# jakovdev/SequenceAligner

Hardware: AMD Instinct MI355X
Metric: pair-alignments/sec (higher is better)
Workload: dtype u16x2; 1 GPU; cfg2: 10000 protein seqs x U[80,120], nw blosum62 {'gap_pen': 4}, all-vs-all packed triangular; pairs=49995000, cells=501594494441, parallelism=pair-range x1

## Files before the change

sequencealigner_amd/csrc/sa_context.hip:

```cpp
#include <algorithm>
#include <cmath>
#include <cstdio>
#include <cstdlib>
#include <cstring>

#include "sa_ctx.h"

bool sa_device_ready(int device)
{
	int count = 0;
	hipError_t err = hipGetDeviceCount(&count);
	if (err != hipSuccess || count <= 0) {
		sa_set_error("No HIP devices available (%s); libseqalign_hip has no CPU fallback",
			     err == hipSuccess ? "device count is 0" : hipGetErrorString(err));
		return false;
	}
	if (device < 0 || device >= count) {
		sa_set_error("HIP device %d out of range (%d visible)", device, count);
		return false;
	}
	SA_HIP_CHECK(hipSetDevice(device), return false);
	return true;
}

// ... 234 lines not shown
}

extern "C" sa_ctx *sa_ctx_create(int device, struct sa_input in, const struct sa_scoring *sc)
{
	return sa_guard("sa_ctx_create", (sa_ctx *)nullptr, [&] { return ctx_create_impl(device, in, sc); });
}

extern "C" void sa_ctx_destroy(sa_ctx *ctx)
{
	if (!ctx)
		return;
	(void)hipSetDevice(ctx->device);
	for (auto &ev : ctx->events) {
		(void)hipEventDestroy(ev.e0);
		(void)hipEventDestroy(ev.e1);
	}
	sa_plan_release(ctx);
	sa_deliver_release(ctx);
	for (auto &ar : ctx->arranged) {
		(void)hipFree(ar.d_codes);
		(void)hipFree(ar.d_off);
		(void)hipFree(ar.d_rowmap);
		(void)hipFree(ar.d_posmap);
	}
	(void)hipFree(ctx->d_codes);
	(void)hipFree(ctx->d_meta);
	(void)hipFree(ctx->d_off);
	(void)hipFree(ctx->d_sub);
	(void)hipFree(ctx->d_sub8);
	(void)hipFree(ctx->d_scratch);
	(void)hipFree(ctx->d_counters);
	for (hipEvent_t ev : ctx->slot_done)
		if (ev)
			(void)hipEventDestroy(ev);
	(void)hipFree(ctx->d_long_scratch);
	for (int k = 0; k < sa_ctx::NSIDE; k++) {
		if (ctx->side[k])
			(void)hipStreamDestroy(ctx->side[k]);
		if (ctx->join_ev[k])
			(void)hipEventDestroy(ctx->join_ev[k]);
	}
	if (ctx->fork_ev)
		(void)hipEventDestroy(ctx->fork_ev);
	delete ctx;
}

// ... 32 lines not shown
	do {
		SA_HIP_CHECK(hipMalloc(&ar.d_codes, codes_s.size()), break);
		SA_HIP_CHECK(hipMalloc(&ar.d_off, sizeof(int32_t) * off_s.size()), break);
		SA_HIP_CHECK(hipMalloc(&ar.d_rowmap, sizeof(int32_t) * rowmap.size()), break);
		SA_HIP_CHECK(hipMalloc(&ar.d_posmap, sizeof(int32_t) * posmap.size()), break);
		SA_HIP_CHECK(hipMemcpy(ar.d_codes, codes_s.data(), codes_s.size(), hipMemcpyHostToDevice), break);
		SA_HIP_CHECK(hipMemcpy(ar.d_off, off_s.data(), sizeof(int32_t) * off_s.size(), hipMemcpyHostToDevice), break);
		SA_HIP_CHECK(hipMemcpy(ar.d_rowmap, rowmap.data(), sizeof(int32_t) * rowmap.size(), hipMemcpyHostToDevice), break);
		SA_HIP_CHECK(hipMemcpy(ar.d_posmap, posmap.data(), sizeof(int32_t) * posmap.size(), hipMemcpyHostToDevice), break);
		ctx->arranged.push_back(ar);
		ok = true;
	} while (0);
	if (!ok) {
		(void)hipFree(ar.d_codes);
		(void)hipFree(ar.d_off);
		(void)hipFree(ar.d_rowmap);
		(void)hipFree(ar.d_posmap);
		return false;
	}
	*out = &ctx->arranged.back();
	return true;
}

extern "C" void sa_ctx_timing(sa_ctx *ctx, int enable)
{
	if (!ctx)
		return;
	(void)hipSetDevice(ctx->device);
	for (auto &ev : ctx->events) {
		(void)hipEventDestroy(ev.e0);
		(void)hipEventDestroy(ev.e1);
	}
	ctx->events.clear();
	ctx->timing = enable != 0;
}

static int timing_read_impl(sa_ctx *ctx, char *kernel_name, int cap, int64_t *launches, double *total_ms,
			    int64_t *pairs, int64_t *cells, double *all_kernels_ms)
{
	if (!ctx)
		return 1;
	(void)hipSetDevice(ctx->device);
	struct Acc {
		double ms = 0;
		int64_t n = 0, pairs = 0, cells = 0;
	};
// ... 45 lines not shown
```

sequencealigner_amd/csrc/sa_ctx.h:

```cpp
#ifndef SA_CTX_H
#define SA_CTX_H

#include <atomic>
#include <chrono>
#include <deque>
#include <exception>
#include <memory>
#include <new>
#include <string>
#include <vector>

#include "sa_env.h"
#include "sa_guard.h"
#include "sa_internal.h"
#include "sa_plan.h"

struct sa_ctx {
	int device = 0;
	int32_t num = 0, max_len = 0, min_len = 0;
	int64_t pairs = 0;
	sa_scoring sc{};
	SaEnv env;
	std::vector<sa_meta> meta;
	std::vector<int32_t> off;
// ... 10 lines not shown
	unsigned *d_counters = nullptr;
	uint64_t call_no = 0;
	hipEvent_t slot_done[COUNTER_SLOTS] = {};
	bool slot_dirty[COUNTER_SLOTS] = {};
	int32_t *d_long_scratch = nullptr;
	int64_t long_stride = 0;
	int long_wgs = 0;
	int persistent_wgs = 0;
	enum { NSIDE = 8 };
	hipStream_t side[NSIDE] = {};
	hipEvent_t fork_ev = nullptr, join_ev[NSIDE] = {};
	bool sys_ok = false;
	int32_t sys_pconst = 0, sys_q = 0;
	int64_t sys_gain = 0, sys_slack = 0;
	int pk_kmax = 0, pk16_kmax = 0;
	int pk16_f16_kmax = 0;
	int pk_chunk_cap = SA_SYS_CHUNK;
	int32_t pk_pconst = 0, pk_q = 0, pk_floor = 0;
	int64_t pk_gain = 0, pk_slack = 0, pk_extra = 0;
	struct Arranged {
		SaArrKey key;
		uint8_t *d_codes = nullptr;
		int32_t *d_off = nullptr, *d_rowmap = nullptr, *d_posmap = nullptr;
	};
	std::deque<Arranged> arranged;
	bool out_is_host = false;
	struct Plan {
		SaHostPlan h;
		struct DevClass {
			int32_t *d_jlist = nullptr, *d_tprefix = nullptr, *d_tlist = nullptr;
			int64_t *d_doff = nullptr;
		};
		struct DevBundle {
			SaPkClassArgs *d_args = nullptr;
			uint32_t *d_ulist = nullptr;
		};
		std::vector<DevClass> dc;
		std::vector<DevBundle> db;
		SaPlaceSeg *d_segs = nullptr;
		int32_t nsegs = 0;
		uint64_t stamp = 0;
	};
	std::vector<std::unique_ptr<Plan>> plans;
	Plan *plan = nullptr;
	uint64_t plan_clock = 0;
	bool timing = false;
// ... 13 lines not shown
		double encode = 0, device = 0, upload = 0, code_objects = 0, pin = 0, plan = 0, arrange = 0;
	} setup;
	struct Deliver {
		hipStream_t compute = nullptr, copy = nullptr;
		hipEvent_t done[2] = {}, copied[2] = {};
		int32_t *d_buf[2] = {};
		int64_t buf_elems[2] = {};
		int32_t *h_stage[2] = {};
		int64_t stage_elems[2] = {};
		int32_t *d_packed = nullptr, *d_full = nullptr;
		int64_t packed_elems = 0, full_elems = 0;
		unsigned *h_counters = nullptr;
		int64_t h_counters_n = 0;
	} dl;
};

static inline double sa_ms_since(std::chrono::steady_clock::time_point t0)
{
	return std::chrono::duration<double, std::milli>(std::chrono::steady_clock::now() - t0).count();
}

bool sa_device_ready(int device);
bool sa_arranged_store(sa_ctx *ctx, const SaArrKey &key, const sa_ctx::Arranged **out);
SaPlanInputs sa_plan_inputs(const sa_ctx *ctx);

void sa_plan_release(sa_ctx *ctx);
bool sa_plan_get(sa_ctx *ctx, int64_t start, int64_t count, int world, bool share_host);
bool sa_prepare_range(sa_ctx *ctx, int64_t start, int64_t count, bool host_out);
int sa_align_range_impl(sa_ctx *ctx, int64_t start, int64_t count, int32_t *d_scores, void *stream, bool out16,
			int world = 0, int rank = 0, int32_t *host_out = nullptr);

void sa_deliver_release(sa_ctx *ctx);
bool sa_host_range_is_pinned(const void *p, size_t bytes);
size_t sa_host_available_bytes();
bool sa_host_range_in_malloc_heap(const void *p, size_t bytes);

bool sa_progress_wanted();
void sa_report_progress(double fraction);
void sa_progress_speaker(bool here);
int sa_devices_in_use(const SaEnv &env);

bool sa_align_gathered(struct sa_input in, struct sa_output out, const struct sa_scoring *sc, const int *devices, int ndev,
		       double *phase_seconds, double *breakdown_ms);
bool sa_rccl_available(std::string *why);

#endif
// ... 1 lines not shown
```

sequencealigner_amd/csrc/sa_env.cpp:

```cpp
#include "sa_env.h"

#include <algorithm>
#include <cstdlib>

static bool flag(const char *name) { return getenv(name) != nullptr; }
static int number(const char *name, int fallback, int lo, int hi)
{
	const char *v = getenv(name);
	if (!v || !*v)
		return fallback;
	return std::max(lo, std::min(hi, atoi(v)));
}

SaEnv sa_env_read()
{
	SaEnv e;
	e.force_generic = flag("SA_HIP_FORCE_GENERIC");
	e.no_pk = flag("SA_HIP_NO_PK");
	e.no_pk16 = flag("SA_HIP_NO_PK16");
	e.no_sort = flag("SA_HIP_NO_SORT");
	e.concurrent_classes = flag("SA_HIP_CONCURRENT_CLASSES");
	e.one_tile_size = flag("SA_HIP_ONE_TILE_SIZE");
	e.chunk = number("SA_HIP_CHUNK", 0, 1, 32);
	e.pk_wgs = number("SA_HIP_PK_WGS", 0, 0, 1 << 20);
	e.stagger = number("SA_HIP_STAGGER", 0, 0, 64);
	e.rotate_prio = getenv("SA_HIP_ROTATE_PRIO") ? (atoi(getenv("SA_HIP_ROTATE_PRIO")) != 0) : -1;
	e.small_below = number("SA_HIP_SMALL_BELOW", 16, 0, 1 << 20);
	e.small_div = number("SA_HIP_SMALL_DIV", 4, 2, 64);
	e.small_frac = number("SA_HIP_SMALL_FRAC", 5, 2, 1 << 20);
	e.no_pin = flag("SA_HIP_NO_PIN");
	e.no_direct = flag("SA_HIP_NO_DIRECT");
	e.no_shells = flag("SA_HIP_NO_SHELLS");
	e.devices = number("SA_HIP_DEVICES", 0, 0, 1024);
	e.split = number("SA_HIP_SPLIT", 0, 0, 1024);
	e.gather = getenv("SA_HIP_GATHER") ? (atoi(getenv("SA_HIP_GATHER")) != 0) : -1;
	e.tiles_split = number("SA_HIP_TILES_SPLIT", 0, 0, 64);
	e.verbose = flag("SA_HIP_VERBOSE");
	e.stamps = flag("SA_HIP_STAMPS");
	e.stamps_dump = getenv("SA_HIP_STAMPS_DUMP");
	e.ztrace = flag("SA_HIP_ZTRACE");
	return e;
}
```

sequencealigner_amd/csrc/sa_env.h:

```cpp
#ifndef SA_ENV_H
#define SA_ENV_H

struct SaEnv {
	bool force_generic = false;
	bool no_pk = false;
	bool no_pk16 = false;
	bool no_sort = false;
	bool concurrent_classes = false;
	bool one_tile_size = false;
	int chunk = 0;
	int pk_wgs = 0;
	int stagger = 0;
	int rotate_prio = -1;
	int small_below = 16;
	int small_div = 4;
	int small_frac = 5;
	bool no_pin = false;
	bool no_direct = false;
	bool no_shells = false;
	int devices = 0;
	int split = 0;
	int gather = -1;
	int tiles_split = 0;
	bool verbose = false;
	bool stamps = false;
	const char *stamps_dump = nullptr;
	bool ztrace = false;
};

SaEnv sa_env_read();
// ... 3 lines not shown
```

sequencealigner_amd/csrc/sa_launch.hip:

```cpp
#include <algorithm>
#include <cstdio>
#include <cstring>

#include "sa_ctx.h"


static void plan_free_device(sa_ctx::Plan &pl)
{
	for (auto &c : pl.dc) {
		(void)hipFree(c.d_jlist);
		(void)hipFree(c.d_tprefix);
		(void)hipFree(c.d_tlist);
		(void)hipFree(c.d_doff);
	}
	(void)hipFree(pl.d_segs);
	for (auto &b : pl.db) {
		(void)hipFree(b.d_args);
		(void)hipFree(b.d_ulist);
	}
	pl.dc.clear();
	pl.db.clear();
	pl.d_segs = nullptr;
}

void sa_plan_release(sa_ctx *ctx)
{
	for (auto &pl : ctx->plans)
		plan_free_device(*pl);
	ctx->plans.clear();
	ctx->plan = nullptr;
}

template <typename T> static bool upload(T *&dst, const std::vector<T> &v)
{
	SA_HIP_CHECK(hipMalloc(reinterpret_cast<void **>(&dst), sizeof(T) * std::max<size_t>(v.size(), 1)), return false);
	if (!v.empty()) {
		SA_HIP_CHECK(hipMemcpy(dst, v.data(), sizeof(T) * v.size(), hipMemcpyHostToDevice), return false);
	}
	return true;
}

static bool resolve_levels(sa_ctx *ctx, const SaArrKey (&keys)[SA_PK_SORT_LEVELS], SaArranged (&lv)[SA_PK_SORT_LEVELS])
{
	for (int l = 0; l < SA_PK_SORT_LEVELS; l++) {
		lv[l] = SaArranged{};
		if (!keys[l].block)
			continue;
		const sa_ctx::Arranged *ar = nullptr;
		if (!sa_arranged_store(ctx, keys[l], &ar))
			return false;
		if (ar)
			lv[l] = { ar->d_codes, ar->d_off, ar->d_rowmap, ar->d_posmap, ar->key.block };
	}
	return true;
}

static bool plan_upload(sa_ctx *ctx, sa_ctx::Plan &pl)
{
	const SaHostPlan &h = pl.h;
	pl.dc.resize(h.classes.size());
	for (size_t ci = 0; ci < h.classes.size(); ci++) {
		const auto &cl = h.classes[ci];
		auto &d = pl.dc[ci];
		if (!upload(d.d_jlist, cl.jlist) || !upload(d.d_tprefix, cl.tprefix))
			return false;
		if (h.world >= 1 && (!upload(d.d_tlist, cl.tlist) || !upload(d.d_doff, cl.doff)))
			return false;
	}
	if (h.world >= 1 && !h.segs.empty()) {
		std::vector<SaPlaceSeg> segs(h.segs.size());
		for (size_t k = 0; k < h.segs.size(); k++) {
			const SaHostSeg &hs = h.segs[k];
			SaPlaceSeg &sg = segs[k];
			sg = SaPlaceSeg{};
			sg.src = hs.src;
// ... 7 lines not shown
			if (hs.map_kind) {
				const sa_ctx::Arranged *ar = nullptr;
				if (!sa_arranged_store(ctx, hs.key, &ar))
					return false;
				if (!ar) {
					sa_set_error("plan: placement names an arranged copy the store does not have");
					return false;
				}
				sg.map = hs.map_kind == 2 ? ar->d_posmap : ar->d_rowmap;
			}
		}
		if (!upload(pl.d_segs, segs))
			return false;
		pl.nsegs = (int32_t)segs.size();
	}
	pl.db.resize(h.bundles.size());
	for (size_t bi = 0; bi < h.bundles.size(); bi++) {
		const auto &b = h.bundles[bi];
		std::vector<SaPkClassArgs> args(b.args.size());
		for (size_t x = 0; x < b.args.size(); x++) {
			const SaHostPkArgs &ha = b.args[x];
			SaPkClassArgs &a = args[x];
			a = SaPkClassArgs{};
			if (!resolve_levels(ctx, ha.lv, a.lv))
				return false;
			const auto &d = pl.dc[(size_t)ha.cls_index];
			a.jlist = d.d_jlist;
			a.tprefix = d.d_tprefix;
			a.dense_off = h.world >= 1 ? d.d_doff : nullptr;
			a.ncols = ha.ncols;
			a.npart = ha.npart;
			a.k = ha.k;
			a.delta = ha.delta;
			a.pk_base = ha.pk_base;
			a.chunk = ha.chunk;
		}
		if (!upload(pl.db[bi].d_args, args) || !upload(pl.db[bi].d_ulist, b.ulist))
			return false;
	}
	return true;
}

bool sa_plan_get(sa_ctx *ctx, int64_t start, int64_t count, int world, bool share_host)
{
	for (auto &pl : ctx->plans)
		if (pl->h.start == start && pl->h.count == count && pl->h.world == world && pl->h.share_host == share_host) {
			pl->stamp = ++ctx->plan_clock;
// ... 511 lines not shown
```

sequencealigner_amd/csrc/sa_plan.cpp:

```cpp
#include "sa_plan.h"
#include "sa_guard.h"

#include <algorithm>
#include <cmath>
#include <cstdlib>

int32_t sa_column_of(int64_t p)
{
	int64_t j = (int64_t)((1.0 + std::sqrt(1.0 + 8.0 * (double)p)) * 0.5);
	while (j * (j - 1) / 2 > p)
		--j;
	while ((j + 1) * j / 2 <= p)
		++j;
	return (int32_t)j;
}

SaPairPlan::SaPairPlan(const sa_meta *m, int32_t n) : num(n), pairs((int64_t)n * (n - 1) / 2), meta(m)
{
	len_prefix.assign((size_t)n + 1, 0);
	cell_prefix.assign((size_t)n + 1, 0);
	for (int32_t k = 0; k < n; k++) {
		len_prefix[(size_t)k + 1] = len_prefix[(size_t)k] + m[k].len;
		cell_prefix[(size_t)k + 1] = cell_prefix[(size_t)k] + (int64_t)m[k].len * len_prefix[(size_t)k];
	}
// ... 82 lines not shown
	for (int32_t b0 = 0; b0 + block <= num; b0 += block) {
		for (int32_t k = 0; k < block; k++)
			idx[(size_t)k] = b0 + k;
		std::stable_sort(idx.begin(), idx.end(), [&](int32_t a, int32_t b) { return meta[a].len > meta[b].len; });
		rounds.clear();
		rest.clear();
		for (int32_t k = 0; k < block;) {
			int32_t e = k;
			while (e < block && meta[idx[(size_t)e]].len == meta[idx[(size_t)k]].len)
				e++;
			const int32_t pure = (e - k) / ng * ng;
			rounds.insert(rounds.end(), idx.begin() + k, idx.begin() + k + pure);
			rest.insert(rest.end(), idx.begin() + k + pure, idx.begin() + e);
			k = e;
		}
		rounds.insert(rounds.end(), rest.begin(), rest.end());
		for (int32_t r = 0; r < block / ng; r++) {
			const int32_t pass = r / slots, w = r % slots;
			const int32_t slot = (pass & 1) ? slots - 1 - w : w;
			for (int g = 0; g < ng; g++) {
				const int gg = (pass & 1) ? ng - 1 - g : g;
				rowmap[(size_t)(b0 + slot * wave_rows + gg * ch + pass)] = rounds[(size_t)(r * ng + g)];
			}
		}
	}
}

static const char *const TOO_LARGE = "packed range too large for one launch; split it into smaller ranges";

bool sa_plan_host(const SaPlanInputs &in, int64_t start, int64_t count, int world, bool share_host, SaHostPlan &plan)
{
	plan = SaHostPlan();
	const int32_t num = in.num;
	const int64_t all_pairs = (int64_t)num * (num - 1) / 2;
	if (num < 2 || !in.meta || start < 0 || count <= 0 || start > all_pairs - count || world < 0 || world > 1024) {
		sa_set_error("plan: bad range [%lld,+%lld) of %lld pairs or world %d", (long long)start, (long long)count,
			     (long long)all_pairs, world);
		return false;
	}
	const int64_t end = start + count;
	std::vector<std::vector<int32_t>> jl((size_t)SA_PLAN_NCLASSES), tp((size_t)SA_PLAN_NCLASSES);
	std::vector<int64_t> cpairs((size_t)SA_PLAN_NCLASSES, 0), ccells((size_t)SA_PLAN_NCLASSES, 0);
	std::vector<std::vector<std::pair<int32_t, int32_t>>> rows_of((size_t)SA_PLAN_NCLASSES);
	std::vector<int64_t> lenpre((size_t)num + 1, 0);
	for (int32_t k = 0; k < num; k++)
		lenpre[(size_t)k + 1] = lenpre[(size_t)k] + in.meta[k].len;
// ... 414 lines not shown
```

sequencealigner_amd/csrc/sa_plan.h:

```cpp
#ifndef SA_PLAN_H
#define SA_PLAN_H

#include <cstdint>
#include <string>
#include <utility>
#include <vector>

#include "sa_shapes.h"

int32_t sa_column_of(int64_t p);
inline int64_t sa_tri(int64_t j) { return j * (j - 1) / 2; }

struct SaPairPlan {
	int32_t num = 0;
	int64_t pairs = 0;
	const sa_meta *meta = nullptr;
	std::vector<int64_t> len_prefix;
	std::vector<int64_t> cell_prefix;
	SaPairPlan(const sa_meta *m, int32_t n);
	int64_t cells_before(int64_t p) const;
};

struct SaArrKey {
	int ng = 0, ch = 0;
// ... 23 lines not shown
	bool sys_ok = false;
	int32_t sys_pconst = 0, sys_q = 0;
	int64_t sys_gain = 0, sys_slack = 0;
	int pk_kmax = 0, pk16_kmax = 0, pk16_f16_kmax = 0, pk_chunk_cap = SA_SYS_CHUNK;
	int32_t pk_pconst = 0, pk_q = 0, pk_floor = 0;
	int64_t pk_gain = 0, pk_slack = 0, pk_extra = 0;
};
SaKernelLimits sa_kernel_limits(const sa_scoring &sc, int32_t max_len, int32_t min_len, bool force_generic, bool no_pk, bool no_pk16);

int32_t sa_pk_delta(const SaPlanInputs &in, int g, int k);
int32_t sa_pk_base(const SaPlanInputs &in, int g, int k);

struct SaPkCls {
	bool small;
	int g, k;
};
SaPkCls sa_pk_decode(int cls);
int sa_systolic_class_for(int32_t n);

bool sa_arranged_exists(int32_t num, const SaArrKey &key);
int sa_pk_arranged_keys(const SaPlanInputs &in, int pk_g, int pk_k, int32_t chunk_pk, bool host_out, SaArrKey (&lv)[SA_PK_SORT_LEVELS]);
void sa_arrange_rows(const sa_meta *meta, int32_t num, const SaArrKey &key, std::vector<int32_t> &rowmap);

struct SaHostClass {
	int cls = 0;
	int32_t ncols = 0, ntiles = 0;
	int32_t npart = 0;
	int32_t chunk = 0;
	int64_t pairs = 0, cells = 0;
	std::vector<int32_t> jlist, tprefix;
	std::vector<int32_t> part_rows;
	std::vector<int32_t> tlist;
	std::vector<int64_t> doff;
	std::vector<int16_t> owner;
	std::vector<int32_t> rank_first;
	std::vector<int64_t> rank_pairs, rank_cells;
};

struct SaHostSeg {
	int64_t src, dst;
	int32_t count, pos0, ia, ib, flags;
	int map_kind;
	SaArrKey key;
};

struct SaHostPkArgs {
// ... 39 lines not shown
```

sequencealigner_amd/csrc/sa_shapes.h:

```cpp
#ifndef SA_SHAPES_H
#define SA_SHAPES_H

#include <cstdint>

#include "../../include/seqalign_hip.h"

#if defined(__HIPCC__)
#define SA_HD __host__ __device__
#else
#define SA_HD
#endif

enum : int { SA_CODE_SEP = 24, SA_CODE_NOP = 25, SA_CODE_ROWS = 26 };

void sa_set_error(const char *fmt, ...) __attribute__((format(printf, 1, 2)));


#define SA_SYS_CHUNK 32
#define SA_SYS_WPB(G, LONG) ((G) >= 32 ? 4 : 1)
#define SA_SYS_CLASS_LIST(X) \
	X(0, 8, 1) X(1, 8, 2) X(2, 8, 3) X(3, 8, 4) \
	X(4, 8, 5) X(5, 8, 6) X(6, 8, 7) X(7, 8, 8) \
	X(8, 8, 9) X(9, 8, 10) X(10, 8, 11) X(11, 8, 12) \
	X(12, 8, 13) X(13, 8, 14) X(14, 8, 15) X(15, 8, 16) \
// ... 29 lines not shown
#define SA_PK_K_LIST(X) \
	X(1) X(2) X(3) X(4) X(5) X(6) X(7) X(8) X(9) X(10) X(11) X(12) \
	X(13) X(14) X(15) X(16) X(17) X(18) X(19) X(20) X(21) X(22) X(23) X(24)
#define SA_PK_K16_MIN 13
#define SA_PK16_KMAX 64
#define SA_PK16_F16_KMAX 52
#define SA_PK_K16_LIST(X) \
	X(13) X(14) X(15) X(16) X(17) X(18) X(19) X(20) X(21) X(22) X(23) X(24) X(25) X(26) \
	X(27) X(28) X(29) X(30) X(31) X(32) X(33) X(34) X(35) X(36) X(37) X(38) X(39) X(40) \
	X(41) X(42) X(43) X(44) X(45) X(46) X(47) X(48) X(49) X(50) X(51) X(52) X(53) X(54) \
	X(55) X(56) X(57) X(58) X(59) X(60) X(61) X(62) X(63) X(64)
enum : int { SA_PK_CLASS0 = SA_SYS_NCLASSES + 1, SA_PK16_CLASS0 = SA_PK_CLASS0 + SA_PK_KMAX + 1,
	     SA_PK_CLASSES_END = SA_PK16_CLASS0 + SA_PK16_KMAX + 1,
	     SA_PK_SMALL = SA_PK_CLASSES_END - SA_PK_CLASS0,
	     SA_PLAN_NCLASSES = SA_PK_CLASSES_END + SA_PK_SMALL };

#define SA_PK_BUNDLE 8
struct SaArranged {
	const uint8_t *codes;
	const int32_t *off;
	const int32_t *rowmap;
	const int32_t *posmap;
	int32_t rows;
};
struct SaPkClassArgs {
	const int32_t *jlist;
	const int32_t *tprefix;
	const int64_t *dense_off;
	int32_t ncols, npart, k;
	int32_t delta, pk_base;
	int32_t chunk;
	SaArranged lv[SA_PK_SORT_LEVELS];
};
#define SA_PK_UTILE_BITS 28
SA_HD constexpr int sa_pk_lds_fixed(int g, int wpb) { return 416 * wpb * (64 / g); }
SA_HD constexpr int sa_pk_lds_bytes(int method, int g, int k) { return sa_pk_lds_fixed(g, sa_pk_wpb(method, g, k)) + SA_CODE_ROWS * ((k + 3) / 4) * 256; }
inline int sa_pk_bundle_klo(int g, int k) { return g == 8 ? 1 + (k - 1) / SA_PK_BUNDLE * SA_PK_BUNDLE : SA_PK_K16_MIN + (k - SA_PK_K16_MIN) / SA_PK_BUNDLE * SA_PK_BUNDLE; }


#define SA_SHARE_PAD(rows) (((rows) + 7) & ~7)

SA_HD inline int sa_pk_pick_level(const int32_t *lvrows, int32_t ra, int32_t rb, int32_t i_begin, int32_t tile_rows)
{
	int pick = -1;
	if (ra % tile_rows != 0)
		return pick;
	for (int l = SA_PK_SORT_LEVELS - 1; l >= 0; l--) {
		const int32_t sr = lvrows[l];
		if (sr <= 0)
			continue;
		const int32_t blk0 = i_begin / sr * sr;
		if (blk0 >= ra && blk0 + sr <= rb)
			pick = l;
	}
	return pick;
}

struct SaPlaceSeg {
	int64_t src;
// ... 9 lines not shown
```

sequencealigner_amd/csrc/sa_systolic_pk.inc:

```
#include "sa_internal.h"
#include <atomic>
#include <type_traits>
#if !defined(SA_PK_G) || (SA_PK_G != 8 && SA_PK_G != 16)
#error "define SA_PK_G (8 or 16) before including sa_systolic_pk.inc"
#endif
#if SA_PK_G == 16 && !defined(SA_PK16_PART)
#error "define SA_PK16_PART (0: K = 13..44, 1: K = 45..64) before including sa_systolic_pk.inc with SA_PK_G 16"
#endif

#define SA_PK_STORE(nt, v, p)                          \
	do {                                           \
		if (nt) {                              \
			asm volatile("");  \
			__builtin_nontemporal_store((v), (p)); \
		} else                                 \
			*(p) = (v);                    \
	} while (0)

#ifndef SA_PK_OPAQUE_TOKEN
#define SA_PK_OPAQUE_TOKEN 1
#endif
#ifndef SA_PK_QUIET_BLOCKS
#define SA_PK_QUIET_BLOCKS 0
#endif
// ... 38 lines not shown
	const uint32_t lo = __builtin_amdgcn_readfirstlane((uint32_t)v), hi = __builtin_amdgcn_readfirstlane((uint32_t)(v >> 32));
	typedef __attribute__((address_space(1))) T *global_ptr;
	return (T *)reinterpret_cast<global_ptr>(((uint64_t)hi << 32) | lo);
}

__device__ __forceinline__ int32_t uload(const int32_t *p) { return __builtin_amdgcn_readfirstlane(*p); }

template <int METHOD, int G, int K, bool F16>
__device__ __forceinline__ void pk_tile(const SaSysArgs &A, const int32_t t_raw, const int32_t ntiles)
{
	static_assert(G == 8 || G == 16, "packed kernels: 8- or 16-lane groups");
	constexpr int NG = 64 / G, WPB = sa_pk_wpb(METHOD, G, K), NGW = NG * WPB;
	constexpr int W = G * K;
	constexpr int PARTS = (K + 3) / 4;
	constexpr int NSLOT = G;
	constexpr int COPIES = 16 / G;
	constexpr int PARTSTRIDE = COPIES * NSLOT * 16;
	static_assert(PARTSTRIDE == 256, "a part spans all 64 banks");
	constexpr int ROWSTRIDE = PARTS * PARTSTRIDE;
	constexpr int PROF_BYTES = SA_CODE_ROWS * ROWSTRIDE;
	constexpr int TSHIFT = (SA_CODE_ROWS - 1) * ROWSTRIDE < 65536 ? 0 : 8;
	constexpr uint32_t TUNIT = (uint32_t)ROWSTRIDE >> TSHIFT;
	static_assert((SA_CODE_ROWS - 1) * TUNIT < 65536, "the token of a profile row must fit u16");
	uint8_t *const s_prof = sa_pk_lds + sa_pk_lds_fixed(G, WPB);
	static_assert(PROF_BYTES + sa_pk_lds_fixed(G, WPB) == sa_pk_lds_bytes(METHOD, G, K), "host and kernel agree on the LDS of a class");
	constexpr int OUT_HALFS = 2 * NG * CH;
	static_assert(WPB * OUT_HALFS * 2 >= SA_SUB_DIM * SA_SUB_DIM, "the staged matrix must fit the score storage");
	int16_t *const s_out_all = reinterpret_cast<int16_t *>(sa_pk_lds);
	constexpr int RING = 64;
	constexpr int GSTRIDE = 2 * RING + 16;
	uint16_t *const s_ring_all = reinterpret_cast<uint16_t *>(sa_pk_lds + WPB * OUT_HALFS * 2);
	static_assert(WPB * OUT_HALFS * 2 + WPB * NG * GSTRIDE * 2 == sa_pk_lds_fixed(G, WPB), "LDS carve");
	static_assert(sa_pk_lds_fixed(G, WPB) % 256 == 0, "the profile starts on a 256-byte boundary: a part spans all 64 banks");

	int lane_id = threadIdx.x;
	asm volatile("" : "+v"(lane_id));
	const int lane = lane_id & 63;
	const int wv = __builtin_amdgcn_readfirstlane(lane_id >> 6);
	int16_t *s_out = s_out_all + wv * OUT_HALFS;
	uint16_t *s_ring = s_ring_all + wv * (NG * GSTRIDE);
	const int lig = G == 8 ? (lane & 15) >> 1 : lane & 15;
	const int grp = G == 8 ? (lane >> 4) * 2 + (lane & 1) : lane >> 4;
	const int copy = G == 8 ? lane & 1 : 0;
	const bool leader = lig == 0;

	const bool active = t_raw < ntiles;
// ... 7 lines not shown
	int32_t ia[2], ib[2], offj[2], nh[2], pad[2];
#pragma unroll
	for (int h = 0; h < 2; h++) {
		const int32_t j = jh[h];
		tri[h] = (int64_t)j * (j - 1) / 2;
		const int64_t a = A.start > tri[h] ? A.start - tri[h] : 0;
		const int64_t b = A.end - tri[h] < j ? A.end - tri[h] : j;
		ia[h] = (int32_t)a;
		ib[h] = (int32_t)(b > a ? b : a);
		offj[h] = uload(A.off + j);
		nh[h] = uload(A.off + j + 1) - offj[h] - 1;
		pad[h] = W - nh[h];
	}
	const int32_t ra = ia[0] < ia[1] ? ia[0] : ia[1], rb = ib[0] > ib[1] ? ib[0] : ib[1];
	const int32_t chunk = t < nfull ? t - uload(A.tprefix + lo) : uload(A.tprefix + lo + 1) - uload(A.tprefix + lo);
	const int32_t ch_full = A.chunk;
	const int32_t i_begin = ra + chunk * (NGW * ch_full);
	const int32_t i_count = rb - i_begin < NGW * ch_full ? rb - i_begin : NGW * ch_full;
	const int32_t ch = (i_count + NGW - 1) / NGW;
	const int gw = wv * NG;
	const uint8_t *rcodes = A.codes;
	const int32_t *roff = A.off, *rowmap = nullptr, *posmap = nullptr;
	int32_t sort_rows = 0;
	{
		const int32_t lvrows[SA_PK_SORT_LEVELS] = { uload(&A.lvp[0].rows), uload(&A.lvp[1].rows), uload(&A.lvp[2].rows),
							    uload(&A.lvp[3].rows) };
		static_assert(SA_PK_SORT_LEVELS == 4, "lvrows lists four levels");
		const int l = sa_pk_pick_level(lvrows, ra, rb, i_begin, NGW * ch_full);
		if (l >= 0) {
			const SaArranged &L = A.lvp[l];
			rcodes = uniform_ptr(L.codes);
			roff = uniform_ptr(L.off);
			rowmap = uniform_ptr(L.rowmap);
			posmap = uniform_ptr(L.posmap);
			sort_rows = lvrows[0];
#pragma unroll
			for (int k = 1; k < SA_PK_SORT_LEVELS; k++)
				if (l == k)
					sort_rows = lvrows[k];
		}
	}
	const bool sorted = sort_rows > 0;

	int8_t *const sub = reinterpret_cast<int8_t *>(s_out_all);
	for (int k = lane_id; k < SA_SUB_DIM * SA_SUB_DIM; k += 64 * WPB)
		sub[k] = A.sub8[k];
	uint8_t *const s_cols = reinterpret_cast<uint8_t *>(s_ring_all);
	static_assert(2 * W <= WPB * NG * GSTRIDE * 2, "the staged columns fit the ring storage");
	for (int k = lane_id; k < 2 * W; k += 64 * WPB) {
		const int h = k >= W, c0 = k - h * W - pad[h];
		s_cols[k] = c0 >= 0 ? A.codes[offj[h] + c0] : (uint8_t)0xff;
	}
	__syncthreads();

	{
		constexpr int BUILDERS = NGW / COPIES;
		constexpr int ROWS_EACH = (SA_CODE_ROWS + BUILDERS - 1) / BUILDERS;
		const int a_lo = ((gw + grp) / COPIES) * ROWS_EACH;
		uint8_t *const slot = s_prof + copy * (NSLOT * 16) + lig * 16;
#pragma unroll 4
		for (int q = 0; q < K; q++) {
			int bq[2];
#pragma unroll
			for (int h = 0; h < 2; h++) {
				const int c = (int)s_cols[h * W + lig * K + q];
				bq[h] = c == 0xff ? -1 : c;
			}
#pragma unroll
			for (int r = 0; r < ROWS_EACH; r++) {
				const int a = a_lo + r;
				if (a >= SA_CODE_ROWS)
					break;
				uint32_t v = 0;
#pragma unroll
				for (int h = 0; h < 2; h++) {
					int e = 0;
					if (a < SA_SUB_DIM && bq[h] >= 0) {
						e = (int)sub[a * SA_SUB_DIM + bq[h]] + A.pconst;
						if (METHOD == SA_METHOD_GA && pad[h] != 0 && lig * K + q == pad[h])
							e -= A.q;
					}
					v |= (uint32_t)(e & 0xffff) << (16 * h);
				}
				*reinterpret_cast<uint32_t *>(slot + a * ROWSTRIDE + (q >> 2) * PARTSTRIDE + (q & 3) * 4) = v;
			}
		}
	}

	const int32_t ib_g = i_begin + (gw + grp) * ch;
	int32_t cnt_g = i_count - (gw + grp) * ch;
	cnt_g = cnt_g < 0 ? 0 : cnt_g > ch ? ch : cnt_g;
	const int32_t sbeg = roff[ib_g < A.num ? ib_g : 0];
	const int32_t slen = cnt_g > 0 ? roff[ib_g + cnt_g] - sbeg : 0;
	int32_t smax = 0;
#pragma unroll
	for (int g = 0; g < NG; g++) {
		int32_t c = i_count - (gw + g) * ch;
		c = c < 0 ? 0 : c > ch ? ch : c;
		const int32_t b = i_begin + (gw + g) * ch;
		const int32_t l = c > 0 ? roff[b + c] - roff[b] : 0;
		smax = l > smax ? l : smax;
	}
	const int32_t steps = smax + G - 1;
	const int32_t nblk = (steps + 15) >> 4;
	const int32_t last = slen > 0 ? slen - 1 : 0;
	const int r16 = lane & 15;
	constexpr int TPL = G == 8 ? 2 : 1;
	auto fpos = [&](int u) -> int { return G == 8 ? (r16 & ~1) + u : r16; };
	const uint32_t ulast = (uint32_t)(sbeg + last);
	auto load_block = [&](int32_t blk, int u) -> int {
		const uint32_t at = (uint32_t)(sbeg + fpos(u)) + (uint32_t)(blk << 4);
		return (int)rcodes[at < ulast ? at : ulast];
	};
	constexpr uint32_t SEPWORD = (uint32_t)SA_CODE_SEP * TUNIT;
	constexpr uint32_t NOPWORD = (uint32_t)SA_CODE_NOP * TUNIT;
	auto block_word = [&](int32_t blk, int raw, int u) -> uint32_t {
		const int32_t pos = (blk << 4) + fpos(u);
		return pos < slen ? (uint32_t)raw * TUNIT : NOPWORD;
	};
	uint16_t *ring = s_ring + grp * GSTRIDE;
	auto ring_write = [&](int32_t blk, uint32_t word, int u) {
		const int i0 = ((blk << 4) + fpos(u)) & (RING - 1);
		ring[i0] = (uint16_t)word;
		ring[i0 + RING] = (uint16_t)word;
	};
	auto fold16 = [&](unsigned long long m) -> uint32_t {
		m |= m >> 32;
		m |= m >> 16;
		return (uint32_t)m & 0xffffu;
	};
	auto block_events = [&](const uint32_t (&w)[TPL], uint32_t &mine) -> uint32_t {
		if (G == 16) {
			const unsigned long long m = __ballot(w[0] == SEPWORD);
			mine = (uint32_t)(m >> (lane & 48)) & 0xffffu;
			return fold16(m);
		}
		uint32_t any = 0;
		mine = 0;
#pragma unroll
		for (int u = 0; u < TPL; u++) {
			const unsigned long long m = __ballot(w[u] == SEPWORD);
			const uint32_t f = fold16(m);
			any |= ((f | (f >> 1)) & 0x5555u) << u;
			mine |= ((uint32_t)(m >> ((lane & 48) + (lane & 1))) & 0x5555u) << u;
		}
		return any;
	};

	const uint32_t base2 = pk2((uint32_t)A.pk_base);
	const uint32_t delta2 = pk2((uint32_t)A.delta);
	const uint32_t q2 = pk2((uint32_t)-A.q);
	const uint32_t cmask2 = (pad[0] == 0 ? 0xffffu : 0u) | (pad[1] == 0 ? 0xffff0000u : 0u);
	uint32_t V[K], Y[K];
	uint32_t vl[2];
	uint32_t xout = 0;
	uint32_t vbase;
	uint32_t fl = 0;
	uint32_t flead = 0, xlead = 0;
	uint32_t best = 0, carry = 0;
	const uint32_t e2 = pk2((uint32_t)-A.gap_e);
	const uint32_t gqs2 = pk2((uint32_t)(A.gap_e - A.gap_o));
	int32_t frame = 0;
	int nsep = 0;
	const uint32_t inj0 = METHOD == SA_METHOD_NW ? base2 : base2 - 2 * q2;
	vl[0] = vl[1] = vbase = inj0;
	if (METHOD == SA_METHOD_SW) {
		const uint32_t o2 = pk2((uint32_t)-A.gap_o);
		const uint32_t top = base2 - o2 - (uint32_t)lig * e2;
		vl[0] = base2 - o2 - e2;
// ... 3 lines not shown
		flead = base2;
		fl = base2 - (uint32_t)(lig + 1) * e2;
		best = base2 - (uint32_t)lig * e2;
#pragma unroll
		for (int q = 0; q < K; q++)
			V[q] = top, Y[q] = top;
	} else if (METHOD == SA_METHOD_NW) {
#pragma unroll
		for (int q = 0; q < K; q++)
			V[q] = base2, Y[q] = 0;
	} else {
		xout = base2 - q2;
#pragma unroll
		for (int q = 0; q < K; q++)
			V[q] = inj0, Y[q] = inj0;
	}

	__syncthreads();
	for (int k = lane; k < NG * GSTRIDE; k += 64)
		s_ring[k] = (uint16_t)NOPWORD;
	__syncthreads();
	unsigned long long ev_lo = METHOD == SA_METHOD_GA ? 1ull << 63 : 0ull, ev_hi;
	uint32_t gm, gmask;
	{
		uint32_t w0[TPL];
#pragma unroll
		for (int u = 0; u < TPL; u++) {
			w0[u] = block_word(0, load_block(0, u), u);
			ring_write(0, w0[u], u);
		}
		ev_hi = block_events(w0, gmask);
		gm = (gmask << 2) | (METHOD == SA_METHOD_GA ? 2u : 0u);
	}
	int raw_next[TPL];
#pragma unroll
	for (int u = 0; u < TPL; u++)
		raw_next[u] = load_block(1, u);
	const uint8_t *const lane_prof = s_prof + copy * (NSLOT * 16) + lig * 16;
	auto ring_base = [&](int32_t blk) -> const uint16_t * { return ring + (((blk << 4) - lig) & (RING - 1)); };
	auto prof_row = [&](uint32_t word, uint4 (&P)[PARTS]) {
		const uint8_t *row = lane_prof + (word << TSHIFT);
#pragma unroll
		for (int p = 0; p < PARTS; p++)
			P[p] = *reinterpret_cast<const uint4 *>(row + p * PARTSTRIDE);
	};
	const uint16_t *rb0 = ring_base(0);
	uint32_t tk_cur = rb0[0], tk_nxt = rb0[1];
	uint4 P[PARTS];
	prof_row(tk_cur, P);

	auto do_block = [&](const int32_t blk) __attribute__((always_inline)) {
		if (A.rotate_prio) {
			switch (((uint32_t)A.rotate_prio + (uint32_t)blk) & 3u) {
			case 0: __builtin_amdgcn_s_setprio(0); break;
			case 1: __builtin_amdgcn_s_setprio(1); break;
			case 2: __builtin_amdgcn_s_setprio(2); break;
			default: __builtin_amdgcn_s_setprio(3); break;
			}
		}
		const unsigned long long ev_in =
			METHOD == SA_METHOD_GA ? (ev_hi | (ev_hi << 1) | (ev_hi << 2) | (ev_lo >> 63) | (ev_lo >> 62)) : ev_hi;
		const uint32_t ev = (uint32_t)(((ev_lo >> (64 - (G - 1))) | (ev_hi << (G - 1)) | ev_in) & 0xffffu);
		uint32_t wn[TPL], gmask_next;
#pragma unroll
		for (int u = 0; u < TPL; u++) {
			wn[u] = block_word(blk + 1, raw_next[u], u);
			ring_write(blk + 1, wn[u], u);
		}
		const uint32_t evn = block_events(wn, gmask_next);
#pragma unroll
		for (int u = 0; u < TPL; u++)
			raw_next[u] = load_block(blk + 2, u);
		const uint16_t *rbase = ring_base(blk);

		auto step = [&](auto has_events, const int s) __attribute__((always_inline)) {
			uint32_t &vcur = vl[s & 1];
			if (METHOD == SA_METHOD_SW)
				carry = pkmax(shift_in<G>(0u, carry), best);
			if (decltype(has_events)::value && __builtin_expect((ev >> s) & 1u, 0)) {
				asm volatile("" ::: "memory");
				if ((gm >> (s + 2)) & 1u) {
#pragma unroll
					for (int q = 0; q < K; q++) {
						V[q] = pksubsat(V[q], delta2);
						if (METHOD != SA_METHOD_NW)
							Y[q] = pksubsat(Y[q], delta2);
					}
					if (METHOD != SA_METHOD_NW)
						xout = pksubsat(xout, delta2);
					if (METHOD == SA_METHOD_SW) {
						fl = pksubsat(fl, delta2);
						best = pksubsat(best, delta2);
						carry = pksubsat(carry, delta2);
					}
					if (!leader) {
// ... 160 lines not shown
					}
				}
				xout = x;
			}
			tk_cur = tk_nxt;
#if SA_PK_OPAQUE_TOKEN
			uint32_t tk_wide = tk_far;
			asm volatile("" : "+v"(tk_wide));
			tk_nxt = tk_wide;
#else
			tk_nxt = tk_far;
#endif
		};
		constexpr bool QUIET = SA_PK_QUIET_BLOCKS && METHOD == SA_METHOD_NW && G == 8 && K <= 16;
		if (QUIET && ev == 0) {
#pragma unroll
			for (int s = 0; s < 16; s++)
				step(std::false_type{}, s);
		} else {
#pragma unroll
			for (int s = 0; s < 16; s++)
				step(std::true_type{}, s);
		}
		gm = (gmask_next << 2) | (gm >> 16);
		ev_lo = (ev_lo >> 16) | (ev_hi << 48);
		ev_hi = evn;
	};
	const unsigned long long ph1 = A.stamps ? __builtin_amdgcn_s_memtime() : 0ull;
	for (int32_t blk2 = 0; blk2 < nblk; blk2 += 2) {
		do_block(blk2);
		if (blk2 + 1 < nblk)
			do_block(blk2 + 1);
	}
	if (A.stamps && threadIdx.x == 0) {
		A.stamps[3 * (size_t)A.nlocal + 3 * (size_t)A.stamp_u + 0] = ph1;
		A.stamps[3 * (size_t)A.nlocal + 3 * (size_t)A.stamp_u + 1] = __builtin_amdgcn_s_memtime();
		A.stamps[3 * (size_t)A.nlocal + 3 * (size_t)A.stamp_u + 2] = (unsigned long long)nblk * 16;
	}
	__syncthreads();

	if (A.dense_off) {
		const int64_t draw = A.dense_off[t];
		const int64_t dbase = (int64_t)(((uint64_t)(uint32_t)__builtin_amdgcn_readfirstlane((int32_t)(draw >> 32)) << 32) |
						(uint32_t)__builtin_amdgcn_readfirstlane((int32_t)draw));
		const int32_t cntp = SA_SHARE_PAD(i_count);
#pragma unroll
		for (int g = 0; g < NG; g++) {
			int32_t c = i_count - (gw + g) * ch;
			c = c < 0 ? 0 : c > ch ? ch : c;
			if (lane < c && active) {
				const int32_t is = i_begin + (gw + g) * ch + lane;
				const int32_t m = roff[is + 1] - roff[is] - 1;
#pragma unroll
				for (int h = 0; h < 2; h++) {
					if (h == 1 && dup)
						continue;
					const int32_t raw = s_out[h * NG * CH + g * CH + lane];
					int32_t score;
					if (METHOD == SA_METHOD_NW)
						score = raw + (m + nh[h]) * A.gap_g;
// ... 259 lines not shown
```

Before: 3.439 billion pair-alignments/s.

## Precompute token streams and event masks on host for sorted G=8 packed kernel

```diff
diff --git a/sequencealigner_amd/csrc/sa_context.hip b/sequencealigner_amd/csrc/sa_context.hip
--- a/sequencealigner_amd/csrc/sa_context.hip
+++ b/sequencealigner_amd/csrc/sa_context.hip
@@ -280,6 +280,11 @@
 		(void)hipFree(ar.d_off);
 		(void)hipFree(ar.d_rowmap);
 		(void)hipFree(ar.d_posmap);
+		for (auto &tk : ar.tokens) {
+			(void)hipFree(tk.d_tok);
+			(void)hipFree(tk.d_ev);
+			(void)hipFree(tk.d_toff);
+		}
 	}
 	(void)hipFree(ctx->d_codes);
 	(void)hipFree(ctx->d_meta);
@@ -358,6 +363,69 @@
 	return true;
 }
 
+bool sa_arranged_tokens(sa_ctx *ctx, const SaArrKey &key, uint32_t tunit, const sa_ctx::Arranged::Tokens **out)
+{
+	*out = nullptr;
+	sa_ctx::Arranged *ar = nullptr;
+	for (auto &a : ctx->arranged)
+		if (a.key == key)
+			ar = &a;
+	if (!ar)
+		return true;
+	for (const auto &tk : ar->tokens)
+		if (tk.tunit == tunit) {
+			*out = tk.d_tok ? &tk : nullptr;
+			return true;
+		}
+	const auto t_arr = std::chrono::steady_clock::now();
+	struct Acc {
+		sa_ctx *c;
+		std::chrono::steady_clock::time_point t;
+		~Acc() { c->setup.arrange += sa_ms_since(t); }
+	} acc{ ctx, t_arr };
+	const int32_t num = ctx->num;
+	std::vector<int32_t> rowmap, off_s((size_t)num + 1);
+	sa_arrange_rows(ctx->meta.data(), num, key, rowmap);
+	std::vector<uint8_t> codes_s(ctx->codes.size());
+	off_s[0] = 0;
+	for (int32_t p = 0; p < num; p++) {
+		const int32_t i = rowmap[(size_t)p];
+		const int32_t n = ctx->off[(size_t)i + 1] - ctx->off[(size_t)i];
+		memcpy(codes_s.data() + off_s[(size_t)p], ctx->codes.data() + ctx->off[(size_t)i], (size_t)n);
+		off_s[(size_t)p + 1] = off_s[(size_t)p] + n;
+	}
+	SaTokenCopy tc;
+	sa_token_copy(codes_s.data(), off_s.data(), num, key, tunit, tc);
+	sa_ctx::Arranged::Tokens tk;
+	tk.tunit = tunit;
+	if (tc.tok.empty() || tc.tok.size() >= ((size_t)1 << 30)) {
+		ar->tokens.push_back(tk);
+		return true;
+	}
+	bool ok = false;
+	do {
+		SA_HIP_CHECK(hipMalloc(&tk.d_tok, sizeof(uint16_t) * tc.tok.size()), break);
+		SA_HIP_CHECK(hipMalloc(&tk.d_ev, sizeof(uint32_t) * tc.ev.size()), break);
+		SA_HIP_CHECK(hipMalloc(&tk.d_toff, sizeof(int32_t) * tc.toff.size()), break);
+		SA_HIP_CHECK(hipMemcpy(tk.d_tok, tc.tok.data(), sizeof(uint16_t) * tc.tok.size(), hipMemcpyHostToDevice), break);
+		SA_HIP_CHECK(hipMemcpy(tk.d_ev, tc.ev.data(), sizeof(uint32_t) * tc.ev.size(), hipMemcpyHostToDevice), break);
+		SA_HIP_CHECK(hipMemcpy(tk.d_toff, tc.toff.data(), sizeof(int32_t) * tc.toff.size(), hipMemcpyHostToDevice), break);
+		ar->tokens.push_back(tk);
+		ok = true;
+	} while (0);
+	if (ok && ctx->env.verbose)
+		fprintf(stderr, "[seqalign_hip] token form of arranged copy (%d,%d,%d), unit %u: %zu words, %zu streams\n", key.ng, key.ch,
+			key.block, tunit, tc.tok.size(), tc.toff.size() - 1);
+	if (!ok) {
+		(void)hipFree(tk.d_tok);
+		(void)hipFree(tk.d_ev);
+		(void)hipFree(tk.d_toff);
+		return false;
+	}
+	*out = &ar->tokens.back();
+	return true;
+}
+
 extern "C" void sa_ctx_timing(sa_ctx *ctx, int enable)
 {
 	if (!ctx)
diff --git a/sequencealigner_amd/csrc/sa_ctx.h b/sequencealigner_amd/csrc/sa_ctx.h
--- a/sequencealigner_amd/csrc/sa_ctx.h
+++ b/sequencealigner_amd/csrc/sa_ctx.h
@@ -56,6 +56,13 @@
 		SaArrKey key;
 		uint8_t *d_codes = nullptr;
 		int32_t *d_off = nullptr, *d_rowmap = nullptr, *d_posmap = nullptr;
+		struct Tokens {
+			uint32_t tunit = 0;
+			uint16_t *d_tok = nullptr;
+			uint32_t *d_ev = nullptr;
+			int32_t *d_toff = nullptr;
+		};
+		std::vector<Tokens> tokens;
 	};
 	std::deque<Arranged> arranged;
 	bool out_is_host = false;
@@ -115,6 +122,7 @@
 
 bool sa_device_ready(int device);
 bool sa_arranged_store(sa_ctx *ctx, const SaArrKey &key, const sa_ctx::Arranged **out);
+bool sa_arranged_tokens(sa_ctx *ctx, const SaArrKey &key, uint32_t tunit, const sa_ctx::Arranged::Tokens **out);
 SaPlanInputs sa_plan_inputs(const sa_ctx *ctx);
 
 void sa_plan_release(sa_ctx *ctx);
diff --git a/sequencealigner_amd/csrc/sa_env.cpp b/sequencealigner_amd/csrc/sa_env.cpp
--- a/sequencealigner_amd/csrc/sa_env.cpp
+++ b/sequencealigner_amd/csrc/sa_env.cpp
@@ -19,6 +19,7 @@
 	e.no_pk = flag("SA_HIP_NO_PK");
 	e.no_pk16 = flag("SA_HIP_NO_PK16");
 	e.no_sort = flag("SA_HIP_NO_SORT");
+	e.no_tokens = flag("SA_HIP_NO_TOKENS");
 	e.concurrent_classes = flag("SA_HIP_CONCURRENT_CLASSES");
 	e.one_tile_size = flag("SA_HIP_ONE_TILE_SIZE");
 	e.chunk = number("SA_HIP_CHUNK", 0, 1, 32);
diff --git a/sequencealigner_amd/csrc/sa_env.h b/sequencealigner_amd/csrc/sa_env.h
--- a/sequencealigner_amd/csrc/sa_env.h
+++ b/sequencealigner_amd/csrc/sa_env.h
@@ -6,6 +6,7 @@
 	bool no_pk = false;
 	bool no_pk16 = false;
 	bool no_sort = false;
+	bool no_tokens = false;
 	bool concurrent_classes = false;
 	bool one_tile_size = false;
 	int chunk = 0;
diff --git a/sequencealigner_amd/csrc/sa_launch.hip b/sequencealigner_amd/csrc/sa_launch.hip
--- a/sequencealigner_amd/csrc/sa_launch.hip
+++ b/sequencealigner_amd/csrc/sa_launch.hip
@@ -40,7 +40,7 @@
 	return true;
 }
 
-static bool resolve_levels(sa_ctx *ctx, const SaArrKey (&keys)[SA_PK_SORT_LEVELS], SaArranged (&lv)[SA_PK_SORT_LEVELS])
+static bool resolve_levels(sa_ctx *ctx, const SaArrKey (&keys)[SA_PK_SORT_LEVELS], int k, SaArranged (&lv)[SA_PK_SORT_LEVELS])
 {
 	for (int l = 0; l < SA_PK_SORT_LEVELS; l++) {
 		lv[l] = SaArranged{};
@@ -49,8 +49,17 @@
 		const sa_ctx::Arranged *ar = nullptr;
 		if (!sa_arranged_store(ctx, keys[l], &ar))
 			return false;
-		if (ar)
-			lv[l] = { ar->d_codes, ar->d_off, ar->d_rowmap, ar->d_posmap, ar->key.block };
+		if (!ar)
+			continue;
+		lv[l] = { ar->d_codes, ar->d_off, ar->d_rowmap, ar->d_posmap, ar->key.block, nullptr, nullptr, nullptr };
+		const sa_ctx::Arranged::Tokens *tk = nullptr;
+		if (keys[l].ng == 64 / 8 && !ctx->env.no_tokens && !sa_arranged_tokens(ctx, keys[l], sa_pk_tunit(k), &tk))
+			return false;
+		if (tk) {
+			lv[l].tok = tk->d_tok;
+			lv[l].tev = tk->d_ev;
+			lv[l].toff = tk->d_toff;
+		}
 	}
 	return true;
 }
@@ -104,7 +113,7 @@
 			const SaHostPkArgs &ha = b.args[x];
 			SaPkClassArgs &a = args[x];
 			a = SaPkClassArgs{};
-			if (!resolve_levels(ctx, ha.lv, a.lv))
+			if (!resolve_levels(ctx, ha.lv, ha.k, a.lv))
 				return false;
 			const auto &d = pl.dc[(size_t)ha.cls_index];
 			a.jlist = d.d_jlist;
diff --git a/sequencealigner_amd/csrc/sa_plan.cpp b/sequencealigner_amd/csrc/sa_plan.cpp
--- a/sequencealigner_amd/csrc/sa_plan.cpp
+++ b/sequencealigner_amd/csrc/sa_plan.cpp
@@ -128,6 +128,49 @@
 				const int gg = (pass & 1) ? ng - 1 - g : g;
 				rowmap[(size_t)(b0 + slot * wave_rows + gg * ch + pass)] = rounds[(size_t)(r * ng + g)];
 			}
+		}
+	}
+}
+
+void sa_token_copy(const uint8_t *codes, const int32_t *off, int32_t num, const SaArrKey &key, uint32_t tunit, SaTokenCopy &tc)
+{
+	tc = SaTokenCopy();
+	tc.toff.push_back(0);
+	if (!sa_arranged_exists(num, key))
+		return;
+	const int ng = key.ng, g = 64 / key.ng;
+	const int32_t ch = key.ch;
+	const int64_t streams = (int64_t)(num / key.block) * key.block / ch;
+	const uint16_t nop = (uint16_t)(SA_CODE_NOP * tunit);
+	for (int64_t w0 = 0; w0 < streams; w0 += ng) {
+		int32_t smax = 0;
+		for (int64_t s = w0; s < w0 + ng; s++)
+			smax = std::max(smax, off[(s + 1) * ch] - off[s * ch]);
+		const int32_t nblk = (smax + g - 1 + 15) / 16 + 2;
+		const size_t t0 = tc.tok.size(), e0 = tc.ev.size();
+		tc.tok.resize(t0 + (size_t)ng * nblk * 16, nop);
+		tc.ev.resize(e0 + (size_t)ng * nblk * 2, 0);
+		for (int k = 0; k < ng; k++) {
+			const int64_t s = w0 + k;
+			const int32_t beg = off[s * ch], len = off[(s + 1) * ch] - beg;
+			uint16_t *const t = tc.tok.data() + t0 + (size_t)k * nblk * 16;
+			uint32_t *const e = tc.ev.data() + e0 + (size_t)k * nblk * 2;
+			for (int32_t p = 0; p < len; p++)
+				t[p] = (uint16_t)(codes[beg + p] * tunit);
+			for (int64_t q = s * ch; q < (s + 1) * ch; q++) {
+				const int32_t p = off[q + 1] - 1 - beg;
+				e[2 * (p >> 4)] |= 4u << (p & 15);
+			}
+			for (int32_t b = 1; b < nblk; b++)
+				e[2 * b] |= (e[2 * b - 2] >> 16) & 3u;
+			tc.toff.push_back((int32_t)(t0 + (size_t)(k + 1) * nblk * 16));
+		}
+		for (int32_t b = 0; b < nblk; b++) {
+			uint32_t any = 0;
+			for (int k = 0; k < ng; k++)
+				any |= (tc.ev[e0 + (size_t)k * nblk * 2 + 2 * (size_t)b] >> 2) & 0xffffu;
+			for (int k = 0; k < ng; k++)
+				tc.ev[e0 + (size_t)k * nblk * 2 + 2 * (size_t)b + 1] = any;
 		}
 	}
 }
diff --git a/sequencealigner_amd/csrc/sa_plan.h b/sequencealigner_amd/csrc/sa_plan.h
--- a/sequencealigner_amd/csrc/sa_plan.h
+++ b/sequencealigner_amd/csrc/sa_plan.h
@@ -69,6 +69,13 @@
 int sa_pk_arranged_keys(const SaPlanInputs &in, int pk_g, int pk_k, int32_t chunk_pk, bool host_out, SaArrKey (&lv)[SA_PK_SORT_LEVELS]);
 void sa_arrange_rows(const sa_meta *meta, int32_t num, const SaArrKey &key, std::vector<int32_t> &rowmap);
 
+struct SaTokenCopy {
+	std::vector<uint16_t> tok;
+	std::vector<uint32_t> ev;
+	std::vector<int32_t> toff;
+};
+void sa_token_copy(const uint8_t *codes, const int32_t *off, int32_t num, const SaArrKey &key, uint32_t tunit, SaTokenCopy &tc);
+
 struct SaHostClass {
 	int cls = 0;
 	int32_t ncols = 0, ntiles = 0;
diff --git a/sequencealigner_amd/csrc/sa_shapes.h b/sequencealigner_amd/csrc/sa_shapes.h
--- a/sequencealigner_amd/csrc/sa_shapes.h
+++ b/sequencealigner_amd/csrc/sa_shapes.h
@@ -75,6 +75,9 @@
 	const int32_t *rowmap;
 	const int32_t *posmap;
 	int32_t rows;
+	const uint16_t *tok;
+	const uint32_t *tev;
+	const int32_t *toff;
 };
 struct SaPkClassArgs {
 	const int32_t *jlist;
@@ -88,6 +91,8 @@
 #define SA_PK_UTILE_BITS 28
 SA_HD constexpr int sa_pk_lds_fixed(int g, int wpb) { return 416 * wpb * (64 / g); }
 SA_HD constexpr int sa_pk_lds_bytes(int method, int g, int k) { return sa_pk_lds_fixed(g, sa_pk_wpb(method, g, k)) + SA_CODE_ROWS * ((k + 3) / 4) * 256; }
+SA_HD constexpr int sa_pk_tshift(int k) { return (SA_CODE_ROWS - 1) * ((k + 3) / 4) * 256 < 65536 ? 0 : 8; }
+SA_HD constexpr uint32_t sa_pk_tunit(int k) { return (uint32_t)((k + 3) / 4) * 256u >> sa_pk_tshift(k); }
 inline int sa_pk_bundle_klo(int g, int k) { return g == 8 ? 1 + (k - 1) / SA_PK_BUNDLE * SA_PK_BUNDLE : SA_PK_K16_MIN + (k - SA_PK_K16_MIN) / SA_PK_BUNDLE * SA_PK_BUNDLE; }
 
 
diff --git a/sequencealigner_amd/csrc/sa_systolic_pk.inc b/sequencealigner_amd/csrc/sa_systolic_pk.inc
--- a/sequencealigner_amd/csrc/sa_systolic_pk.inc
+++ b/sequencealigner_amd/csrc/sa_systolic_pk.inc
@@ -84,6 +84,7 @@
 	constexpr int TSHIFT = (SA_CODE_ROWS - 1) * ROWSTRIDE < 65536 ? 0 : 8;
 	constexpr uint32_t TUNIT = (uint32_t)ROWSTRIDE >> TSHIFT;
 	static_assert((SA_CODE_ROWS - 1) * TUNIT < 65536, "the token of a profile row must fit u16");
+	static_assert(TSHIFT == sa_pk_tshift(K) && TUNIT == sa_pk_tunit(K), "host (token copies) and kernel agree on the token unit");
 	uint8_t *const s_prof = sa_pk_lds + sa_pk_lds_fixed(G, WPB);
 	static_assert(PROF_BYTES + sa_pk_lds_fixed(G, WPB) == sa_pk_lds_bytes(METHOD, G, K), "host and kernel agree on the LDS of a class");
 	constexpr int OUT_HALFS = 2 * NG * CH;
@@ -137,6 +138,9 @@
 	const uint8_t *rcodes = A.codes;
 	const int32_t *roff = A.off, *rowmap = nullptr, *posmap = nullptr;
 	int32_t sort_rows = 0;
+	const uint16_t *rtok = nullptr;
+	const uint32_t *rtev = nullptr;
+	const int32_t *rtoff = nullptr;
 	{
 		const int32_t lvrows[SA_PK_SORT_LEVELS] = { uload(&A.lvp[0].rows), uload(&A.lvp[1].rows), uload(&A.lvp[2].rows),
 							    uload(&A.lvp[3].rows) };
@@ -148,6 +152,9 @@
 			roff = uniform_ptr(L.off);
 			rowmap = uniform_ptr(L.rowmap);
 			posmap = uniform_ptr(L.posmap);
+			rtok = uniform_ptr(L.tok);
+			rtev = uniform_ptr(L.tev);
+			rtoff = uniform_ptr(L.toff);
 			sort_rows = lvrows[0];
 #pragma unroll
 			for (int k = 1; k < SA_PK_SORT_LEVELS; k++)
@@ -156,6 +163,7 @@
 		}
 	}
 	const bool sorted = sort_rows > 0;
+	const bool tokp = sorted && rtok != nullptr;
 
 	int8_t *const sub = reinterpret_cast<int8_t *>(s_out_all);
 	for (int k = lane_id; k < SA_SUB_DIM * SA_SUB_DIM; k += 64 * WPB)
@@ -202,6 +210,8 @@
 		}
 	}
 
+	auto stream_tile = [&](auto tok_c) __attribute__((always_inline)) {
+	constexpr bool TOK = decltype(tok_c)::value;
 	const int32_t ib_g = i_begin + (gw + grp) * ch;
 	int32_t cnt_g = i_count - (gw + grp) * ch;
 	cnt_g = cnt_g < 0 ? 0 : cnt_g > ch ? ch : cnt_g;
@@ -239,6 +249,17 @@
 		ring[i0] = (uint16_t)word;
 		ring[i0 + RING] = (uint16_t)word;
 	};
+	auto ring_write_tok = [&](int32_t blk, uint32_t words) {
+		const int i0 = ((blk << 4) + fpos(0)) & (RING - 1);
+		if (G == 8) {
+			typedef uint32_t __attribute__((may_alias)) u32_alias;
+			*reinterpret_cast<u32_alias *>(ring + i0) = words;
+			*reinterpret_cast<u32_alias *>(ring + i0 + RING) = words;
+		} else {
+			ring[i0] = (uint16_t)words;
+			ring[i0 + RING] = (uint16_t)words;
+		}
+	};
 	auto fold16 = [&](unsigned long long m) -> uint32_t {
 		m |= m >> 32;
 		m |= m >> 16;
@@ -260,6 +281,17 @@
 			mine |= ((uint32_t)(m >> ((lane & 48) + (lane & 1))) & 0x5555u) << u;
 		}
 		return any;
+	};
+	const int32_t tstream = TOK ? i_begin / ch + gw + grp : 0;
+	const int32_t tbeg = TOK ? rtoff[tstream] : 0;
+	const uint32_t tok_at = 2u * (uint32_t)(tbeg + fpos(0)), tev_at = 8u * (uint32_t)(tbeg >> 4);
+	typedef uint32_t u32x2 __attribute__((ext_vector_type(2)));
+	auto tok_load = [&](int32_t blk) -> uint32_t {
+		const uint8_t *const p = reinterpret_cast<const uint8_t *>(rtok) + (tok_at + ((uint32_t)blk << 5));
+		return G == 8 ? *reinterpret_cast<const uint32_t *>(p) : (uint32_t)*reinterpret_cast<const uint16_t *>(p);
+	};
+	auto tev_load = [&](int32_t blk) -> u32x2 {
+		return *reinterpret_cast<const u32x2 *>(reinterpret_cast<const uint8_t *>(rtev) + (tev_at + ((uint32_t)blk << 3)));
 	};
 
 	const uint32_t base2 = pk2((uint32_t)A.pk_base);
@@ -309,7 +341,20 @@
 	__syncthreads();
 	unsigned long long ev_lo = METHOD == SA_METHOD_GA ? 1ull << 63 : 0ull, ev_hi;
 	uint32_t gm, gmask;
-	{
+	int raw_next[TPL];
+	uint32_t tk_next = 0;
+	u32x2 ev_next = { 0u, 0u };
+	if constexpr (TOK) {
+		ring_write_tok(0, tok_load(0));
+		const u32x2 e0 = tev_load(0);
+		gm = e0.x | (METHOD == SA_METHOD_GA ? 2u : 0u);
+		ev_hi = (uint32_t)__builtin_amdgcn_readfirstlane((int)e0.y);
+		tk_next = tok_load(1);
+		ev_next = tev_load(1);
+#pragma unroll
+		for (int u = 0; u < TPL; u++)
+			raw_next[u] = 0;
+	} else {
 		uint32_t w0[TPL];
 #pragma unroll
 		for (int u = 0; u < TPL; u++) {
@@ -318,11 +363,10 @@
 		}
 		ev_hi = block_events(w0, gmask);
 		gm = (gmask << 2) | (METHOD == SA_METHOD_GA ? 2u : 0u);
-	}
-	int raw_next[TPL];
-#pragma unroll
-	for (int u = 0; u < TPL; u++)
-		raw_next[u] = load_block(1, u);
+#pragma unroll
+		for (int u = 0; u < TPL; u++)
+			raw_next[u] = load_block(1, u);
+	}
 	const uint8_t *const lane_prof = s_prof + copy * (NSLOT * 16) + lig * 16;
 	auto ring_base = [&](int32_t blk) -> const uint16_t * { return ring + (((blk << 4) - lig) & (RING - 1)); };
 	auto prof_row = [&](uint32_t word, uint4 (&P)[PARTS]) {
@@ -348,16 +392,26 @@
 		const unsigned long long ev_in =
 			METHOD == SA_METHOD_GA ? (ev_hi | (ev_hi << 1) | (ev_hi << 2) | (ev_lo >> 63) | (ev_lo >> 62)) : ev_hi;
 		const uint32_t ev = (uint32_t)(((ev_lo >> (64 - (G - 1))) | (ev_hi << (G - 1)) | ev_in) & 0xffffu);
-		uint32_t wn[TPL], gmask_next;
-#pragma unroll
-		for (int u = 0; u < TPL; u++) {
-			wn[u] = block_word(blk + 1, raw_next[u], u);
-			ring_write(blk + 1, wn[u], u);
-		}
-		const uint32_t evn = block_events(wn, gmask_next);
-#pragma unroll
-		for (int u = 0; u < TPL; u++)
-			raw_next[u] = load_block(blk + 2, u);
+		uint32_t gm_next, evn;
+		if constexpr (TOK) {
+			ring_write_tok(blk + 1, tk_next);
+			gm_next = ev_next.x;
+			evn = (uint32_t)__builtin_amdgcn_readfirstlane((int)ev_next.y);
+			tk_next = tok_load(blk + 2);
+			ev_next = tev_load(blk + 2);
+		} else {
+			uint32_t wn[TPL], gmask_next;
+#pragma unroll
+			for (int u = 0; u < TPL; u++) {
+				wn[u] = block_word(blk + 1, raw_next[u], u);
+				ring_write(blk + 1, wn[u], u);
+			}
+			evn = block_events(wn, gmask_next);
+			gm_next = (gmask_next << 2) | (gm >> 16);
+#pragma unroll
+			for (int u = 0; u < TPL; u++)
+				raw_next[u] = load_block(blk + 2, u);
+		}
 		const uint16_t *rbase = ring_base(blk);
 
 		auto step = [&](auto has_events, const int s) __attribute__((always_inline)) {
@@ -564,7 +618,7 @@
 			for (int s = 0; s < 16; s++)
 				step(std::true_type{}, s);
 		}
-		gm = (gmask_next << 2) | (gm >> 16);
+		gm = gm_next;
 		ev_lo = (ev_lo >> 16) | (ev_hi << 48);
 		ev_hi = evn;
 	};
@@ -578,6 +632,15 @@
 		A.stamps[3 * (size_t)A.nlocal + 3 * (size_t)A.stamp_u + 0] = ph1;
 		A.stamps[3 * (size_t)A.nlocal + 3 * (size_t)A.stamp_u + 1] = __builtin_amdgcn_s_memtime();
 		A.stamps[3 * (size_t)A.nlocal + 3 * (size_t)A.stamp_u + 2] = (unsigned long long)nblk * 16;
+	}
+	};
+	if constexpr (G == 8) {
+		if (tokp)
+			stream_tile(std::true_type{});
+		else
+			stream_tile(std::false_type{});
+	} else {
+		stream_tile(std::false_type{});
 	}
 	__syncthreads();
 
```

Result: faster. 3.561 billion pair-alignments/s (median of 6 runs) (+3.6%).
